# autonomousvision/unimatch

Measured on NVIDIA H100. Metric: image-pairs/sec @480x832 gmflow-scale2-refine6; EPE vs reference, higher is better.
Workload: dtype fp32

## Files before the change

### include/unimatch_sm100.h

```cpp
#ifndef UNIMATCH_SM100_H_
#define UNIMATCH_SM100_H_

#include <stdint.h>

#ifdef __cplusplus
extern "C" {
#endif

#define UM_OK 0
#define UM_EINVAL (-22)
#define UM_ECUDA (-5)

#define UM_FEATURE_DIM 128

#define UM_ABI_VERSION 4
int um_abi_version(void);
const char* um_build_info(void);
const char* um_last_error(void);
int64_t um_launch_count(void);

#define UM_MASK_NONE 0
#define UM_MASK_SWIN 1
#define UM_MASK_CAUSAL 2

typedef struct um_attn_geom {
  int32_t h, w;
  int32_t kh, kw;
  int32_t sh, sw;
  int32_t mask_mode;
} um_attn_geom;

int um_window_attention(const float* q, const float* k, const float* v, float* out,
                        int32_t n_streams, int32_t kv_shift,
                        int64_t ldq, int64_t ldk, int64_t ldv, int64_t ldo,
                        const um_attn_geom* geom, void* workspace, int64_t workspace_bytes, int32_t flags,
                        void* stream);
#define UM_ATTN_FORCE_CUDA_CORES 1
int64_t um_window_attention_workspace(const um_attn_geom* geom, int32_t n_streams);

int32_t um_attention_planes_lp(const um_attn_geom* geom);
int um_window_attention_planes(const void* q_planes, const void* k_planes, const void* v_planes, float* out, int64_t ldo,
                               void* out_split, int64_t split_plane_stride, int32_t n_streams, int32_t kv_shift,
                               const um_attn_geom* geom, void* stream);

#define UM_VALUE_TENSOR 0
#define UM_VALUE_COORDS 1
#define UM_VALUE_XCOORD 2
#define UM_POST_NONE 0
#define UM_POST_MINUS_OWN 1
#define UM_POST_OWN_MINUS 2

int um_softmax_expectation(const float* q, const float* k, const float* values, float* out,
                           int32_t n_streams, int32_t n_total, int32_t kv_shift,
                           int64_t ldq, int64_t ldk, int32_t vdim, int32_t value_mode, int32_t post_op,
                           const um_attn_geom* geom, void* workspace, int64_t workspace_bytes, int32_t flags,
                           void* stream);
int64_t um_softmax_expectation_workspace(const um_attn_geom* geom, int32_t n_total, int32_t value_mode);

int um_local_corr_softmax(const float* f0, const float* f1, float* flow,
                          int32_t batch, int32_t h, int32_t w, int32_t ry, int32_t rx, int32_t stereo,
                          void* stream);

int um_local_corr_volume(const float* f0, const float* f1, const float* flow, float* corr,
                         int32_t batch, int32_t h, int32_t w, int32_t radius, int32_t flow_dim, void* stream);

int um_flow_warp(const float* f, const float* flow, float* out,
// ... 211 lines not shown
```

### unimatch_b200/csrc/um_api.cu

```cuda
#include <stdarg.h>

#include <atomic>
#include <initializer_list>

#include <cuda_fp16.h>

#include "um_common.cuh"

namespace um {

static thread_local char g_err[512] = "";
static std::atomic<long long> g_launches{0};

void set_error(const char* fmt, ...) {
  va_list ap;
  va_start(ap, fmt);
  vsnprintf(g_err, sizeof(g_err), fmt, ap);
  va_end(ap);
}
void count_launch(int n) { g_launches.fetch_add(n, std::memory_order_relaxed); }

int window_attention_simt(const float* q, const float* k, const float* v, float* out, int n_streams, int kv_shift,
                          long long ldq, long long ldk, long long ldv, long long ldo, const Geom& g, cudaStream_t st);
bool attention_tc_supported(const Geom& g);
size_t attention_tc_workspace_bytes(const Geom& g, int n_streams);
int window_attention_tc(const float* q, const float* k, const float* v, float* out, int n_streams, int kv_shift,
                        long long ldq, long long ldk, long long ldv, long long ldo, const Geom& g, void* workspace,
                        cudaStream_t st);
int attention_planes_launch(const __half* wq, const __half* wk, const __half* wv, float* out, long long ldo, __half* out_split,
                            long long split_plane, int n_streams, int kv_shift, const Geom& g, cudaStream_t st);
bool expectation_tc_supported(const Geom& g, int value_mode);
size_t expectation_tc_workspace_bytes(const Geom& g, int n_total);
int softmax_expectation_tc(const float* q, const float* k, const float* values, float* out, int n_streams, int n_total,
                           int kv_shift, long long ldq, long long ldk, int vdim, int value_mode, int post_op,
                           const Geom& g, void* workspace, cudaStream_t st);
int softmax_expectation_simt(const float* q, const float* k, const float* values, float* out, int n_streams,
                             int n_total, int kv_shift, long long ldq, long long ldk, int vdim, int value_mode,
                             int post_op, const Geom& g, cudaStream_t st);
int chain_tracks_launch(const float* flow, const float* occ, int n, int h, int w, float* pos, uint8_t* vis, float* pos_out,
                        uint8_t* vis_out, cudaStream_t st);
int track_points_forward_launch(const float* flow, const float* occ, int n, int h, int w, int t0, const float* queries,
                                int nq, int nt, float* pos, uint8_t* vis, float* tracks, uint8_t* visible, cudaStream_t st);
int track_points_backward_launch(const float* flow, const float* occ, int n, int h, int w, const float* queries, int nq,
                                 int nt, float* tracks, uint8_t* visible, cudaStream_t st);

static bool overlap(const void* a, long long abytes, const void* b, long long bbytes) {
  const uintptr_t x = reinterpret_cast<uintptr_t>(a), y = reinterpret_cast<uintptr_t>(b);
  return x < y + (uintptr_t)bbytes && y < x + (uintptr_t)abytes;
}

struct Span {
  const void* p;
  long long bytes;
// ... 33 lines not shown
  um::Geom g;
  if (!um::make_geom(geom, &g) || !um::attention_tc_supported(g)) return 0;
  return (g.lw + 127) / 128 * 128;
}

int um_window_attention_planes(const void* q_planes, const void* k_planes, const void* v_planes, float* out, int64_t ldo,
                               void* out_split, int64_t split_plane_stride, int32_t n_streams, int32_t kv_shift,
                               const um_attn_geom* geom, void* stream) {
  um::Geom g;
  UM_REQUIRE(q_planes && k_planes && v_planes && (out || out_split) && n_streams > 0,
             "um_window_attention_planes: null operand planes / no output / empty batch");
  UM_REQUIRE(um::make_geom(geom, &g), "um_window_attention_planes: bad geometry (h,w must be divisible by kh,kw)");
  UM_REQUIRE(um::attention_tc_supported(g),
             "um_window_attention_planes: geometry not built for the tensor-core kernel (um_attention_planes_lp() == 0)");
  UM_REQUIRE(kv_shift >= 0 && kv_shift < n_streams, "um_window_attention_planes: kv_shift out of range");
  UM_REQUIRE(!out || (ldo % 4 == 0 && ldo >= UM_C), "um_window_attention_planes: ldo must be >= 128 and a multiple of 4");
  UM_REQUIRE(!out_split || (split_plane_stride >= (int64_t)n_streams * g.h * g.w * UM_C && split_plane_stride % 8 == 0),
             "um_window_attention_planes: split_plane_stride must cover n_streams*h*w rows of 128 halves");
  UM_REQUIRE(((reinterpret_cast<uintptr_t>(q_planes) | reinterpret_cast<uintptr_t>(k_planes) |
               reinterpret_cast<uintptr_t>(v_planes) | reinterpret_cast<uintptr_t>(out_split)) & 15) == 0,
             "um_window_attention_planes: planes must be 16-byte aligned");
  return um::attention_planes_launch(reinterpret_cast<const __half*>(q_planes), reinterpret_cast<const __half*>(k_planes),
                                     reinterpret_cast<const __half*>(v_planes), out, ldo, reinterpret_cast<__half*>(out_split),
                                     split_plane_stride, n_streams, kv_shift, g, (cudaStream_t)stream);
}

int um_window_attention(const float* q, const float* k, const float* v, float* out, int32_t n_streams,
                        int32_t kv_shift, int64_t ldq, int64_t ldk, int64_t ldv, int64_t ldo,
                        const um_attn_geom* geom, void* workspace, int64_t workspace_bytes, int32_t flags,
                        void* stream) {
  um::Geom g;
  UM_REQUIRE(q && k && v && out && n_streams > 0, "um_window_attention: null pointer or empty batch");
  UM_REQUIRE(um::make_geom(geom, &g), "um_window_attention: bad geometry (h,w must be divisible by kh,kw)");
  UM_REQUIRE(kv_shift >= 0 && kv_shift < n_streams, "um_window_attention: kv_shift out of range");
  UM_REQUIRE(ldq % 4 == 0 && ldk % 4 == 0 && ldv % 4 == 0 && ldo % 4 == 0 && ldq >= UM_C && ldk >= UM_C &&
                 ldv >= UM_C && ldo >= UM_C,
             "um_window_attention: row strides must be >= 128 and multiples of 4 floats");
  UM_REQUIRE(g.mask_mode >= UM_MASK_NONE && g.mask_mode <= UM_MASK_CAUSAL, "um_window_attention: bad mask_mode");
  cudaStream_t st = (cudaStream_t)stream;
  if (!(flags & UM_ATTN_FORCE_CUDA_CORES) && um::attention_tc_supported(g)) {
    UM_REQUIRE(workspace && workspace_bytes >= (int64_t)um::attention_tc_workspace_bytes(g, n_streams),
               "um_window_attention: workspace too small (%lld bytes needed, see um_window_attention_workspace)",
               (long long)um::attention_tc_workspace_bytes(g, n_streams));
    return um::window_attention_tc(q, k, v, out, n_streams, kv_shift, ldq, ldk, ldv, ldo, g, workspace, st);
  }
  return um::window_attention_simt(q, k, v, out, n_streams, kv_shift, ldq, ldk, ldv, ldo, g, st);
}
// ... 90 lines not shown
```

### unimatch_b200/csrc/um_attention_tc.cu

```cuda
#include <math_constants.h>

#include "um_common.cuh"
#include "um_tc.cuh"

namespace um {

using namespace tc;

namespace {

constexpr int BM = 128, BN = 64;
constexpr int NTHREADS = 288;
constexpr int PRODUCER = 8;
constexpr uint32_t Q_BYTES = 4 * 16384;
constexpr uint32_t KV_STAGE_BYTES = 4 * 8192;
constexpr uint32_t OFF_Q = 0;
constexpr uint32_t OFF_K = OFF_Q + Q_BYTES;
constexpr uint32_t OFF_V = OFF_K + 2 * KV_STAGE_BYTES;
constexpr uint32_t OFF_X = OFF_V + 2 * KV_STAGE_BYTES;
constexpr uint32_t OFF_BAR = OFF_X + 1024;
constexpr uint32_t OFF_KREG = OFF_BAR + 256;
constexpr int MAX_LP = 2048;
constexpr uint32_t SMEM_BYTES = OFF_KREG + MAX_LP;
constexpr float SQRT_C = 11.313708498984761f;
constexpr float EXP_SCALE = 1.4426950408889634f / 11.313708498984761f;
constexpr float LAZY_THRESH = 8.0f / EXP_SCALE;

struct TcParams {
  float* out; long long ldo;
  int n_streams, kv_shift, lp;
  Geom g;
  const float* values; int vdim, value_mode, post_op;
  __half* out_split; long long split_plane;
};

__device__ __forceinline__ uint32_t pack_h2(__half a, __half b) {
  return (uint32_t)__half_as_ushort(a) | ((uint32_t)__half_as_ushort(b) << 16);
}

template <bool HAS_V>
__global__ void __launch_bounds__(NTHREADS, 1)
attn_tc_kernel(const __grid_constant__ CUtensorMap map_q, const __grid_constant__ CUtensorMap map_k,
               const __grid_constant__ CUtensorMap map_v, TcParams p) {
  extern __shared__ __align__(1024) uint8_t smem[];
  uint64_t* bars = reinterpret_cast<uint64_t*>(smem + OFF_BAR);
  uint64_t* q_full = bars + 0;
  uint64_t* k_full = bars + 1;
  uint64_t* k_empty = bars + 3;
  uint64_t* v_full = bars + 5;
  uint64_t* v_empty = bars + 7;
  int8_t* kreg = reinterpret_cast<int8_t*>(smem + OFF_KREG);

  const Geom g = p.g;
  const int warp = threadIdx.x >> 5, lane = threadIdx.x & 31;
  const int m0 = blockIdx.x * BM, win = blockIdx.y, n = blockIdx.z;
  const int nk = (n + p.kv_shift) % p.n_streams;
  const int nwin = g.nwin, lp = p.lp;
  const int T = (g.lw + BN - 1) / BN;
  const int planes = p.n_streams * nwin * lp;

  if (threadIdx.x == 0) {
    mbar_init(q_full, 1);
    for (int i = 0; i < 2; ++i) {
      mbar_init(k_full + i, 1); mbar_init(k_empty + i, 8);
      mbar_init(v_full + i, 1); mbar_init(v_empty + i, 8);
    }
// ... 229 lines not shown
    fence_acc(o);
    __syncwarp();
    if (lane == 0) mbar_arrive(v_empty + s);
  }

  float inv[2];
#pragma unroll
  for (int h = 0; h < 2; ++h) {
    float l = l_run[h];
    l += __shfl_xor_sync(0xffffffffu, l, 1);
    l += __shfl_xor_sync(0xffffffffu, l, 2);
    inv[h] = 1.0f / l;
  }
  consumers_sync();
  float* osm = reinterpret_cast<float*>(smem + OFF_Q);
#pragma unroll
  for (int jj = 0; jj < 16; ++jj)
#pragma unroll
    for (int h = 0; h < 2; ++h) {
      const int row = fr + 8 * h, col = 8 * jj + fc;
      *reinterpret_cast<float2*>(osm + row * 128 + (((col >> 2) ^ (row & 31)) << 2) + (col & 3)) =
          make_float2(o[4 * jj + 2 * h] * inv[h], o[4 * jj + 2 * h + 1] * inv[h]);
    }
  consumers_sync();
  float* obase = p.out + (long long)n * g.h * g.w * p.ldo;
  for (int row = cw * 16; row < cw * 16 + 16; ++row) {
    const int tq = m0 + row;
    if (tq >= g.lw) break;
    const int tk = window_token(g, win, tq);
    const float4 v = *reinterpret_cast<const float4*>(osm + row * 128 + ((lane ^ (row & 31)) << 2));
    if (p.out) *reinterpret_cast<float4*>(obase + (long long)tk * p.ldo + lane * 4) = v;
    if (p.out_split) {
      uint32_t h0, h1, l0, l1;
      split_f16x2(v.x, v.y, &h0, &l0);
      split_f16x2(v.z, v.w, &h1, &l1);
      __half* d = p.out_split + ((long long)n * g.h * g.w + tk) * 128 + lane * 4;
      *reinterpret_cast<uint2*>(d) = make_uint2(h0, h1);
      *reinterpret_cast<uint2*>(d + p.split_plane) = make_uint2(l0, l1);
    }
  }
}

struct SplitParams {
  const float* src[3]; long long ld[3];
  __half* dst[3];
  int n_streams, lp;
  Geom g;
};

__global__ void __launch_bounds__(256) split_windows_kernel(SplitParams p) {
  const Geom g = p.g;
  const int lane = threadIdx.x & 31;
  const int t = blockIdx.x * 8 + (threadIdx.x >> 5);
  const int win = blockIdx.y, n = blockIdx.z;
  if (t >= p.lp) return;
  const long long planes = (long long)p.n_streams * g.nwin * p.lp;
  const long long row = ((long long)n * g.nwin + win) * p.lp + t;
  const int tok = (t < g.lw) ? window_token(g, win, t) : -1;
#pragma unroll
  for (int a = 0; a < 3; ++a) {
    if (!p.src[a]) continue;
// ... 49 lines not shown
}

bool attention_tc_supported(const Geom& g) {
  return g.lw >= BM && padded_lw(g.lw) <= MAX_LP && (g.mask_mode == UM_MASK_NONE || g.mask_mode == UM_MASK_SWIN);
}

size_t attention_tc_workspace_bytes(const Geom& g, int n_streams) {
  return (size_t)3 * 2 * n_streams * g.nwin * padded_lw(g.lw) * 128 * sizeof(__half);
}

int split_windows_launch(const float* q, const float* k, const float* v, long long ldq, long long ldk, long long ldv,
                         __half* wq, __half* wk, __half* wv, int n_streams, const Geom& g, cudaStream_t st, const char* what) {
  SplitParams sp{};
  sp.src[0] = q; sp.src[1] = k; sp.src[2] = v;
  sp.ld[0] = ldq; sp.ld[1] = ldk; sp.ld[2] = ldv;
  sp.dst[0] = wq; sp.dst[1] = wk; sp.dst[2] = wv;
  sp.n_streams = n_streams; sp.lp = padded_lw(g.lw); sp.g = g;
  split_windows_kernel<<<dim3((sp.lp + 7) / 8, g.nwin, n_streams), 256, 0, st>>>(sp);
  return check_launch(what);
}


int attention_planes_launch(const __half* wq, const __half* wk, const __half* wv, float* out, long long ldo, __half* out_split,
                               long long split_plane, int n_streams, int kv_shift, const Geom& g, cudaStream_t st) {
  const int lp = padded_lw(g.lw);
  int rc;
  CUtensorMap mq, mk, mv;
  const uint64_t rows = (uint64_t)2 * n_streams * g.nwin * lp;
  if ((rc = make_map_2d_f16(&mq, wq, rows, 128, BM))) return rc;
  if ((rc = make_map_2d_f16(&mk, wk, rows, 128, BN))) return rc;
  if ((rc = make_map_2d_f16(&mv, wv, rows, 128, BN))) return rc;
  static PerDeviceBytes configured;
  if ((rc = ensure_smem(configured, attn_tc_kernel<true>, SMEM_BYTES, "attn_tc"))) return rc;
  TcParams p{};
  p.out = out; p.ldo = ldo; p.n_streams = n_streams; p.kv_shift = kv_shift; p.lp = lp; p.g = g;
  p.out_split = out_split; p.split_plane = split_plane;
  const int qtiles = (g.lw + BM - 1) / BM;
  attn_tc_kernel<true><<<dim3(qtiles, g.nwin, n_streams), NTHREADS, SMEM_BYTES, st>>>(mq, mk, mv, p);
  return check_launch("um_window_attention(wgmma)");
}

int window_attention_tc(const float* q, const float* k, const float* v, float* out, int n_streams, int kv_shift,
                        long long ldq, long long ldk, long long ldv, long long ldo, const Geom& g, void* workspace,
                        cudaStream_t st) {
  const int lp = padded_lw(g.lw);
  const size_t plane_elems = (size_t)2 * n_streams * g.nwin * lp * 128;
  __half* wq = reinterpret_cast<__half*>(workspace);
  __half* wk = wq + plane_elems;
  __half* wv = wk + plane_elems;
  int rc = split_windows_launch(q, k, v, ldq, ldk, ldv, wq, wk, wv, n_streams, g, st, "um_window_attention(split)");
  if (rc) return rc;
  return attention_planes_launch(wq, wk, wv, out, ldo, nullptr, 0, n_streams, kv_shift, g, st);
}

int softmax_expectation_tc(const float* q, const float* k, const float* values, float* out, int n_streams, int n_total,
                           int kv_shift, long long ldq, long long ldk, int vdim, int value_mode, int post_op,
                           const Geom& g, void* workspace, cudaStream_t st) {
  const int lp = padded_lw(g.lw);
  const size_t plane_elems = (size_t)2 * n_total * g.nwin * lp * 128;
  __half* wq = reinterpret_cast<__half*>(workspace);
  __half* wk = wq + plane_elems;
  int rc = split_windows_launch(q, k, nullptr, ldq, ldk, 0, wq, wk, nullptr, n_total, g, st, "um_softmax_expectation(split)");
  if (rc) return rc;
  CUtensorMap mq, mk;
  const uint64_t rows = (uint64_t)2 * n_total * g.nwin * lp;
  if ((rc = make_map_2d_f16(&mq, wq, rows, 128, BM))) return rc;
  if ((rc = make_map_2d_f16(&mk, wk, rows, 128, BN))) return rc;
  static PerDeviceBytes configured;
  if ((rc = ensure_smem(configured, attn_tc_kernel<false>, SMEM_BYTES, "expect_tc"))) return rc;
  TcParams p{};
  p.out = out; p.ldo = vdim; p.n_streams = n_total; p.kv_shift = kv_shift; p.lp = lp; p.g = g;
  p.values = values; p.vdim = vdim; p.value_mode = value_mode; p.post_op = post_op;
  const int qtiles = (g.lw + BM - 1) / BM;
  attn_tc_kernel<false><<<dim3(qtiles, g.nwin, n_streams), NTHREADS, SMEM_BYTES, st>>>(mq, mk, mk, p);
  return check_launch("um_softmax_expectation(wgmma)");
// ... 4 lines not shown
```

### unimatch_b200/csrc/um_common.cuh

```cuda
#pragma once
#include <cuda_runtime.h>
#include <stdint.h>
#include <stdio.h>

#include "unimatch_sm100.h"

#define UM_STR2(x) #x
#define UM_STR(x) UM_STR2(x)
#define UM_C 128

namespace um {

void set_error(const char* fmt, ...);
void count_launch(int n = 1);

inline int check_launch(const char* what) {
  cudaError_t e = cudaGetLastError();
  if (e != cudaSuccess) {
    set_error("%s: %s", what, cudaGetErrorString(e));
    return UM_ECUDA;
  }
  count_launch();
  return UM_OK;
}
// ... 20 lines not shown
inline int device_sm_count() {
  static int sms[kMaxDevices] = {};
  const int d = current_device();
  if (!sms[d]) {
    int n = 0;
    cudaDeviceGetAttribute(&n, cudaDevAttrMultiProcessorCount, d);
    sms[d] = n > 0 ? n : 132;
  }
  return sms[d];
}

#define UM_REQUIRE(cond, ...)             \
  do {                                    \
    if (!(cond)) {                        \
      um::set_error(__VA_ARGS__);         \
      return UM_EINVAL;                   \
    }                                     \
  } while (0)

struct Geom {
  int h, w, kh, kw, wh, ww, sh, sw, mask_mode, lw, nwin;
};

inline bool make_geom(const um_attn_geom* g, Geom* o) {
  if (!g || g->h <= 0 || g->w <= 0 || g->kh <= 0 || g->kw <= 0) return false;
  if (g->h % g->kh || g->w % g->kw) return false;
  o->h = g->h; o->w = g->w; o->kh = g->kh; o->kw = g->kw;
  o->wh = g->h / g->kh; o->ww = g->w / g->kw;
  o->sh = g->sh; o->sw = g->sw; o->mask_mode = g->mask_mode;
  o->lw = o->wh * o->ww; o->nwin = g->kh * g->kw;
  if (o->sh < 0 || o->sh >= o->h || o->sw < 0 || o->sw >= o->w) return false;
  return true;
}

__device__ __forceinline__ int window_token(const Geom& g, int win, int t, int* yr_out = nullptr, int* xr_out = nullptr) {
  int wy = win / g.kw, wx = win - wy * g.kw;
  int i = t / g.ww, j = t - i * g.ww;
  int yr = wy * g.wh + i, xr = wx * g.ww + j;
  if (yr_out) *yr_out = yr;
  if (xr_out) *xr_out = xr;
  int y = yr + g.sh; if (y >= g.h) y -= g.h;
  int x = xr + g.sw; if (x >= g.w) x -= g.w;
  return y * g.w + x;
}

__device__ __forceinline__ int shift_region(const Geom& g, int yr, int xr) {
// ... 24 lines not shown
```

### unimatch_b200/ops.py

```python
import ctypes
import os

import torch

_HERE = os.path.dirname(os.path.abspath(__file__))
LIB_PATH = os.path.join(_HERE, "libunimatch_sm100.so")

MASK_NONE, MASK_SWIN, MASK_CAUSAL = 0, 1, 2
VALUE_TENSOR, VALUE_COORDS, VALUE_XCOORD = 0, 1, 2
POST_NONE, POST_MINUS_OWN, POST_OWN_MINUS = 0, 1, 2


FORCE_CUDA_CORES = 1
_force_cuda_cores = False


def set_force_cuda_cores(flag):
    global _force_cuda_cores
    _force_cuda_cores = bool(flag)


EVAL_FLOW, EVAL_STEREO, EVAL_DEPTH = 0, 1, 2
EVAL_MASK_ALL, EVAL_MASK_VALID, EVAL_MASK_VALID_MAX = 0, 1, 2
EVAL_PARTS = 128
# ... 39 lines not shown
RAGGED_ITEM_BYTES = ctypes.sizeof(RaggedItem)


class FfnDesc(ctypes.Structure):
    _fields_ = [("src", ctypes.c_void_p * 2), ("src_plane_stride", ctypes.c_int64), ("rows", ctypes.c_int64),
                ("w1", ctypes.c_void_p), ("w2", ctypes.c_void_p), ("hidden", ctypes.c_int32),
                ("residual", ctypes.c_void_p), ("ld_res", ctypes.c_int64), ("gamma", ctypes.c_void_p), ("beta", ctypes.c_void_p),
                ("out_f32", ctypes.c_void_p), ("ld_f32", ctypes.c_int64), ("out_split", ctypes.c_void_p),
                ("split_plane_stride", ctypes.c_int64)]


_P, _I, _L, _F = ctypes.c_void_p, ctypes.c_int32, ctypes.c_int64, ctypes.c_float
_G, _FP, _RC = ctypes.POINTER(AttnGeom), ctypes.POINTER(ctypes.c_float), ctypes.c_int

_SIGNATURES = {
    "um_abi_version": (_RC, []),
    "um_build_info": (ctypes.c_char_p, []),
    "um_last_error": (ctypes.c_char_p, []),
    "um_launch_count": (_L, []),
    "um_window_attention": (_RC, [_P, _P, _P, _P, _I, _I, _L, _L, _L, _L, _G, _P, _L, _I, _P]),
    "um_window_attention_workspace": (_L, [_G, _I]),
    "um_attention_planes_lp": (_I, [_G]),
    "um_window_attention_planes": (_RC, [_P, _P, _P, _P, _L, _P, _L, _I, _I, _G, _P]),
    "um_softmax_expectation": (_RC, [_P, _P, _P, _P, _I, _I, _I, _L, _L, _I, _I, _I, _G, _P, _L, _I, _P]),
    "um_softmax_expectation_workspace": (_L, [_G, _I, _I]),
    "um_local_corr_softmax": (_RC, [_P, _P, _P, _I, _I, _I, _I, _I, _I, _P]),
    "um_local_corr_volume": (_RC, [_P, _P, _P, _P, _I, _I, _I, _I, _I, _P]),
    "um_flow_warp": (_RC, [_P, _P, _P, _I, _I, _I, _I, _P]),
    "um_fb_consistency": (_RC, [_P, _P, _F, _F, _P, _P, _I, _I, _I, _P]),
    "um_fb_consistency_ragged": (_RC, [_P, _L, _P, _F, _F, _P, _L, _P, _I, _I, _I, _P]),
    "um_chain_tracks": (_RC, [_P, _P, _I, _I, _I, _P, _P, _P, _P, _P]),
    "um_track_points_forward": (_RC, [_P, _P, _I, _I, _I, _I, _P, _I, _I, _P, _P, _P, _P, _P]),
    "um_track_points_backward": (_RC, [_P, _P, _I, _I, _I, _P, _I, _I, _P, _P, _P]),
    "um_propagate_local": (_RC, [_P, _P, _P, _P, _I, _I, _I, _I, _I, _L, _L, _P]),
    "um_depth_corr_softmax": (_RC, [_P, _P, _P, _P, _P, _P, _P, _I, _I, _I, _I, _I, _P]),
    "um_add_position": (_RC, [_P, _P, _P, _I, _I, _I, _I, _I, _P]),
    "um_convex_upsample": (_RC, [_P, _P, _P, _I, _I, _I, _I, _I, _F, _P]),
    "um_upsample2x": (_RC, [_P, _P, _I, _I, _I, _I, _F, _P]),
    "um_resize_bilinear": (_RC, [_P, _P, _I, _I, _I, _I, _I, _I, _FP, _I, _P]),
    "um_frames_to_planar": (_RC, [_P, _P, _I, _I, _I, _I, _I, _I, _P]),
    "um_frames_to_planar_ragged": (_RC, [_P, _L, _P, _P, _I, _I, _I, _I, _I, _P]),
    "um_frames_to_planar_normalized": (_RC, [_P, _P, _I, _I, _I, _I, _I, _FP, _FP, _P]),
    "um_frames_to_planar_normalized_ragged": (_RC, [_P, _L, _P, _P, _I, _I, _I, _I, _I, _FP, _FP, _P]),
    "um_resize_bilinear_ragged": (_RC, [_P, _P, _L, _P, _I, _I, _I, _I, _I, _P]),
    "um_disparity_to_image_ragged": (_RC, [_P, _L, _P, _P, _P, _I, _I, _I, _P]),
    "um_flow_to_image": (_RC, [_P, _P, _L, _L, _P, _I, _I, _I, _P]),
# ... 117 lines not shown

def _window_attention_planes(qp, kp, vp, n, kv_shift, h, w, kh, kw, sh, sw, mask_mode, out_f32, out_split):
    g = AttnGeom(h, w, kh, kw, sh, sw, mask_mode)
    lp = int(LIB.um_attention_planes_lp(ctypes.byref(g)))
    if lp == 0:
        raise RuntimeError("window_attention_planes: geometry is not built for the tensor-core kernel")
    for t, nm in ((qp, "q_planes"), (kp, "k_planes"), (vp, "v_planes")):
        _planes_ok(t, nm, n, kh * kw, lp)
    ldo, plane = 0, 0
    if out_f32 is not None:
        ldo = _rows(out_f32, "out_f32")
    if out_split is not None:
        if out_split.dtype != torch.float16 or not out_split.is_contiguous() or out_split.shape[0] != 2 or out_split.shape[-1] != 128:
            raise RuntimeError("window_attention_planes: out_split must be contiguous fp16 planes [2, rows, 128]")
        plane = out_split[0].numel()
    _check(LIB.um_window_attention_planes(_p(qp), _p(kp), _p(vp), _p(out_f32), ldo, _p(out_split), plane, n, kv_shift,
                                          ctypes.byref(g), _stream()), "um_window_attention_planes")


window_attention_planes = _define(
    "window_attention_planes(Tensor q_planes, Tensor k_planes, Tensor v_planes, int n_streams, int kv_shift, int h, int w, "
    "int kh, int kw, int sh, int sw, int mask_mode, Tensor(a!)? out_f32, Tensor(b!)? out_split) -> ()",
    _window_attention_planes)


def _softmax_expectation(q, k, values, n_streams, kv_shift, vdim, value_mode, post_op, h, w, kh, kw, mask_mode):
    ldq, ldk = _rows(q, "q"), _rows(k, "k")
    n_total, l, _ = q.shape
    if values is not None:
        _f32c(values, "values")
    out = torch.empty((n_streams, l, vdim), device=q.device, dtype=torch.float32)
    g = AttnGeom(h, w, kh, kw, 0, 0, mask_mode)
    flags = FORCE_CUDA_CORES if _force_cuda_cores else 0
    ws_bytes = 0 if flags else int(LIB.um_softmax_expectation_workspace(ctypes.byref(g), n_total, value_mode))
    ws = torch.empty((ws_bytes,), device=q.device, dtype=torch.uint8) if ws_bytes else None
    _check(LIB.um_softmax_expectation(_p(q), _p(k), _p(values), _p(out), n_streams, n_total, kv_shift, ldq, ldk, vdim,
                                      value_mode, post_op, ctypes.byref(g), _p(ws), ws_bytes, flags, _stream()),
           "um_softmax_expectation")
    return out


softmax_expectation = _define(
    "softmax_expectation(Tensor q, Tensor k, Tensor? values, int n_streams, int kv_shift, int vdim, int value_mode, "
    "int post_op, int h, int w, int kh, int kw, int mask_mode) -> Tensor", _softmax_expectation)


# ... 646 lines not shown
```

### unimatch_b200/unimatch.py

```python
import math
from collections import namedtuple
from contextlib import contextmanager

import torch
import torch.nn as nn

from . import ops
from .spec import param_spec

_OPS = torch.ops.unimatch_sm100


class _Layer(namedtuple("_Layer", "weights bias kh kw pad_h pad_w stride cout bn mode act gamma beta k")):
    __slots__ = ()

    def out_hw(self, h, w, stride):
        return (h + 2 * self.pad_h - self.kh) // stride + 1, (w + 2 * self.pad_w - self.kw) // stride + 1


def _layer(w, cin_splits, bn, bias=None, act=ops.ACT_NONE, mode=ops.CONV_LINEAR, gamma=None, beta=None, stride=1):
    if w.dim() == 2:
        w = w[:, :, None, None]
    cout, cin, kh, kw = w.shape
    return _Layer(ops.prep_conv_weight(w, cin_splits, (cout + bn - 1) // bn * bn), bias, kh, kw, kh // 2, kw // 2, stride,
# ... 72 lines not shown
        elif ".norm" in key:
            t.fill_(1.0 if key.endswith("weight") else 0.0)
        else:
            t.uniform_(-0.05, 0.05)
        return t

    def train(self, mode=True):
        if mode:
            raise NotImplementedError("unimatch_b200.UniMatch is inference-only (use .eval(); training stays on the reference)")
        return super().train(False)

    def _prepared(self):
        params = dict(self.named_parameters())
        key = (tuple((p._version, p.data_ptr()) for p in params.values()),)
        if self._prep_key == key:
            return self._prep
        w = {k: v.detach() for k, v in params.items()}
        LN = ops.CONV_LN
        P = {"raw": w, "blocks": []}
        for i in range(self.num_transformer_layers):
            sk, ck = "transformer.layers.%d.self_attn." % i, "transformer.layers.%d.cross_attn_ffn." % i
            w_in = torch.cat([w[sk + "q_proj.weight"], w[sk + "k_proj.weight"], w[sk + "v_proj.weight"],
                              w[ck + "k_proj.weight"], w[ck + "v_proj.weight"]], dim=0)
            hid = w[ck + "mlp.0.weight"].shape[0]
            P["blocks"].append(dict(
                tc_in=_layer(w_in, [128], 128),
                tc_m_s=_layer(w[sk + "merge.weight"], [128], 128, mode=LN, gamma=w[sk + "norm1.weight"], beta=w[sk + "norm1.bias"]),
                tc_q_c=_layer(w[ck + "q_proj.weight"], [128], 128),
                tc_m_c=_layer(w[ck + "merge.weight"], [128], 128, mode=LN, gamma=w[ck + "norm1.weight"], beta=w[ck + "norm1.bias"]),
                tc_w1=_layer(w[ck + "mlp.0.weight"], [128, 128], 256, act=ops.ACT_GELU),
                tc_w2=_layer(w[ck + "mlp.2.weight"], [hid], 128, mode=LN, gamma=w[ck + "norm2.weight"], beta=w[ck + "norm2.bias"])))
        P["tcb"] = self._prepare_backbone(w, self.num_scales)
        qw, qb = w["feature_flow_attn.q_proj.weight"], w["feature_flow_attn.q_proj.bias"]
        kw, kb = w["feature_flow_attn.k_proj.weight"], w["feature_flow_attn.k_proj.bias"]
        P["prop_q"] = _layer(qw, [128], 128, qb.contiguous())
        P["prop_k"] = _layer(kw, [128], 128, kb.contiguous())
        P["prop_qk"] = _layer(torch.cat([qw, kw], 0), [128], 128, torch.cat([qb, kb]).contiguous())
        if self.reg_refine:
            P["tc"] = self._prepare_refine(w)
        if "upsampler.0.weight" in w:
            w0 = w["upsampler.0.weight"]
            w0 = torch.cat([w0[:, 2:], w0[:, :2]], dim=1)
            w2 = w["upsampler.2.weight"]
            P["up"] = dict(c0=_layer(w0, [130], 128, w["upsampler.0.bias"], act=ops.ACT_RELU),
                           c2=_layer(w2, [256], 192 if w2.shape[0] % 192 == 0 else 64, w["upsampler.2.bias"]))
        self._prep_key, self._prep = key, P
        return P

    @staticmethod
# ... 181 lines not shown
        if buf is None:
            if len(self._attn_ws) >= 4:
                self._attn_ws.clear()
            buf = torch.zeros((6, 2, n, kh * kw, lp, 128), device=dev, dtype=torch.float16)
            self._attn_ws[key] = buf
        return buf

    def cached_buffers(self):
        return list(self._attn_ws.values()) + list(self._pad_ws.values())

    def _stage_transformer(self, P, x, h, w, attn_type, splits, tag="s0"):
        n, l, c = x.shape
        half = n // 2
        rows = n * l
        rp = _ceil16(rows)
        dev = x.device
        G = self._conv
        mk = torch.empty if rp == rows else torch.zeros
        planes = lambda cp: mk((2, rp, cp), device=dev, dtype=torch.float16)
        f32 = lambda cols: mk((rp, cols), device=dev)
        tok = lambda t, c0, c1: t[:rows].view(n, l, t.shape[-1])[:, :, c0:c1]
        hid = P["blocks"][0]["tc_w1"].cout
        x_f, xo_f, x1_f = f32(c), f32(c), f32(c)
        x_s, xo_s, x1_s, msg_s, m_s = planes(c), planes(c), planes(c), planes(c), planes(c)
        fused_ffn = ops.ffn_tc_supported(rp)
        hid_s = None if fused_ffn else planes(hid)
        x_f[:rows] = x.reshape(rows, c)
        _OPS.split_planes(x_f, x_s, 0)
        y = q_f = None
        for i, blk in enumerate(P["blocks"]):
            geo_s, geo_c = self._attn_plan(attn_type, splits, h, w, i)
            gs, gc = (h, w) + geo_s, (h, w) + geo_c
            lp_s = ops.attention_planes_lp(*gs)
            lp_c = ops.attention_planes_lp(*gc) if geo_c == geo_s else 0
            ws = self._attn_planes(dev, n, h, w, geo_s[0], geo_s[1], lp_s) if lp_s else None
            win_c1 = 640 if lp_c else (384 if lp_s else 0)
            if win_c1 < 640 and y is None:
                y = f32(5 * c)
            G(blk["tc_in"], x_s, rows=rp, out_f32=y if win_c1 < 640 else None, win_dst=ws[:win_c1 // 128] if win_c1 else None,
              win_geom=gs if win_c1 else None, win_c1=win_c1, win_streams=n)
            fl_s, fl_c = (4.0 * (l // (g[0] * g[1])) * l * 128 * n for g in (geo_s, geo_c))
            if lp_s:
                self._timed("attn:" + tag, fl_s, _OPS.window_attention_planes, ws[0], ws[1], ws[2], n, 0, *gs, None, msg_s)
            else:
                msg = self._timed("attn_simt:" + tag, fl_s, _OPS.window_attention, tok(y, 0, 128), tok(y, 128, 256), tok(y, 256, 384), 0, *gs)
                _OPS.split_planes(msg.view(rows, c), msg_s, 0)
            G(blk["tc_m_s"], msg_s, rows=rp, out_f32=x1_f, out_split=x1_s, aux0=x_f)
            if lp_c:
                G(blk["tc_q_c"], x1_s, rows=rp, win_dst=ws[5:6], win_geom=gc, win_c1=128, win_streams=n)
                self._timed("attn:" + tag, fl_c, _OPS.window_attention_planes, ws[5], ws[3], ws[4], n, half, *gc, None, msg_s)
            else:
                if q_f is None:
                    q_f = f32(c)
                G(blk["tc_q_c"], x1_s, rows=rp, out_f32=q_f)
                msg = self._timed("attn_simt:" + tag, fl_c, _OPS.window_attention, tok(q_f, 0, 128), tok(y, 384, 512), tok(y, 512, 640), half, *gc)
                _OPS.split_planes(msg.view(rows, c), msg_s, 0)
            G(blk["tc_m_c"], msg_s, rows=rp, out_split=m_s)
            w1, w2 = blk["tc_w1"], blk["tc_w2"]
            if fused_ffn:
                self._timed("conv", 2.0 * rp * hid * (2 * c + c), _OPS.ffn_tc, x1_s, m_s, w1.weights, w2.weights, x1_f,
                            w2.gamma, w2.beta, xo_f, xo_s, rp)
            else:
                G(w1, x1_s, m_s, rows=rp, out_split=hid_s)
                G(w2, hid_s, rows=rp, out_f32=xo_f, out_split=xo_s, aux0=x1_f)
            x_f, xo_f, x_s, xo_s = xo_f, x_f, xo_s, x_s
        return x_f[:rows].view(n, l, c), x_s

    def _stage_features(self, f0, f1, flow, h, wd, splits):
        Bp, c = f0.shape[0], f0.shape[-1]
        if flow is not None:
            f1 = _OPS.flow_warp(f1.contiguous(), flow.contiguous(), h, wd)
        table = self._pos_table(h // splits, wd // splits, f0.device)
        tok = torch.cat((f0, f1), dim=0).view(2 * Bp, h, wd, c)
        return _OPS.add_position(tok, table, h, wd).view(2 * Bp, h * wd, c)

    def _stage_correlation(self, tok, Bp, h, wd, task, radius, pred_bidir_flow=False, depth=None):
        t0, t1 = tok[:Bp], tok[Bp:]
        if task == "depth":
            cams, from_argmax, bidir = depth
            if bidir:
# ... 280 lines not shown
```

Before: 82.51.

## Fold merge and cross-query projections into weights and fuse LayerNorm into attention

Two weight products are precomputed in fp64 and stored with the fused input projection: merge·v_proj for self and cross attention, and q_proj^T·k_proj for cross attention. The separate merge and cross-query GEMMs disappear from each transformer block. A new attention kernel variant applies LayerNorm, the residual add and split-fp16 output, including a windowed layout that feeds the next attention, directly in its epilogue. This removes several GEMM launches and intermediate buffers per block, at the cost of a heavier epilogue and some numerical drift from the pre-multiplied weights.

```diff
diff --git a/include/unimatch_sm100.h b/include/unimatch_sm100.h
--- a/include/unimatch_sm100.h
+++ b/include/unimatch_sm100.h
@@ -42,6 +42,10 @@
 int um_window_attention_planes(const void* q_planes, const void* k_planes, const void* v_planes, float* out, int64_t ldo,
                                void* out_split, int64_t split_plane_stride, int32_t n_streams, int32_t kv_shift,
                                const um_attn_geom* geom, void* stream);
+int um_window_attention_planes_ln(const void* q_planes, const void* k_planes, const void* v_planes, const float* residual,
+                                  int64_t ld_res, const float* gamma, const float* beta, float* out, int64_t ldo,
+                                  void* out_split, int64_t split_plane_stride, void* out_win, int32_t n_streams,
+                                  int32_t kv_shift, const um_attn_geom* geom, void* stream);
 
 #define UM_VALUE_TENSOR 0
 #define UM_VALUE_COORDS 1
diff --git a/unimatch_b200/csrc/um_api.cu b/unimatch_b200/csrc/um_api.cu
--- a/unimatch_b200/csrc/um_api.cu
+++ b/unimatch_b200/csrc/um_api.cu
@@ -28,7 +28,8 @@
                         long long ldq, long long ldk, long long ldv, long long ldo, const Geom& g, void* workspace,
                         cudaStream_t st);
 int attention_planes_launch(const __half* wq, const __half* wk, const __half* wv, float* out, long long ldo, __half* out_split,
-                            long long split_plane, int n_streams, int kv_shift, const Geom& g, cudaStream_t st);
+                            long long split_plane, int n_streams, int kv_shift, const Geom& g, cudaStream_t st,
+                            const AttnEpilogue& ep);
 bool expectation_tc_supported(const Geom& g, int value_mode);
 size_t expectation_tc_workspace_bytes(const Geom& g, int n_total);
 int softmax_expectation_tc(const float* q, const float* k, const float* values, float* out, int n_streams, int n_total,
@@ -108,7 +109,41 @@
              "um_window_attention_planes: planes must be 16-byte aligned");
   return um::attention_planes_launch(reinterpret_cast<const __half*>(q_planes), reinterpret_cast<const __half*>(k_planes),
                                      reinterpret_cast<const __half*>(v_planes), out, ldo, reinterpret_cast<__half*>(out_split),
-                                     split_plane_stride, n_streams, kv_shift, g, (cudaStream_t)stream);
+                                     split_plane_stride, n_streams, kv_shift, g, (cudaStream_t)stream, um::AttnEpilogue{});
+}
+
+int um_window_attention_planes_ln(const void* q_planes, const void* k_planes, const void* v_planes, const float* residual,
+                                  int64_t ld_res, const float* gamma, const float* beta, float* out, int64_t ldo,
+                                  void* out_split, int64_t split_plane_stride, void* out_win, int32_t n_streams,
+                                  int32_t kv_shift, const um_attn_geom* geom, void* stream) {
+  um::Geom g;
+  UM_REQUIRE(q_planes && k_planes && v_planes && gamma && beta && (out || out_split || out_win) && n_streams > 0,
+             "um_window_attention_planes_ln: null operand planes / gamma / beta, no output or empty batch");
+  UM_REQUIRE(um::make_geom(geom, &g), "um_window_attention_planes_ln: bad geometry (h,w must be divisible by kh,kw)");
+  UM_REQUIRE(um::attention_tc_supported(g),
+             "um_window_attention_planes_ln: geometry not built for the tensor-core kernel (um_attention_planes_lp() == 0)");
+  UM_REQUIRE(kv_shift >= 0 && kv_shift < n_streams, "um_window_attention_planes_ln: kv_shift out of range");
+  UM_REQUIRE(!out || (ldo % 4 == 0 && ldo >= UM_C), "um_window_attention_planes_ln: ldo must be >= 128 and a multiple of 4");
+  UM_REQUIRE(!residual || (ld_res % 4 == 0 && ld_res >= UM_C),
+             "um_window_attention_planes_ln: ld_res must be >= 128 and a multiple of 4");
+  UM_REQUIRE(!out_split || (split_plane_stride >= (int64_t)n_streams * g.h * g.w * UM_C && split_plane_stride % 8 == 0),
+             "um_window_attention_planes_ln: split_plane_stride must cover n_streams*h*w rows of 128 halves");
+  UM_REQUIRE(um::aligned(q_planes, 16) && um::aligned(k_planes, 16) && um::aligned(v_planes, 16) && um::aligned(out_split, 16) &&
+             um::aligned(out_win, 16) && um::aligned(out, 16) && um::aligned(residual, 16) && um::aligned(gamma, 16) &&
+             um::aligned(beta, 16), "um_window_attention_planes_ln: buffers must be 16-byte aligned");
+  const long long rows = (long long)n_streams * g.h * g.w;
+  const long long win_halves = 2LL * n_streams * g.nwin * ((g.lw + 127) / 128 * 128) * UM_C;
+  UM_REQUIRE(um::written_disjoint({{out, out ? ((rows - 1) * ldo + UM_C) * 4 : 0},
+                                   {out_split, out_split ? (split_plane_stride + rows * UM_C) * 2 : 0},
+                                   {out_win, win_halves * 2},
+                                   {residual, residual ? ((rows - 1) * ld_res + UM_C) * 4 : 0},
+                                   {q_planes, win_halves * 2}, {k_planes, win_halves * 2}, {v_planes, win_halves * 2}}, 3),
+             "um_window_attention_planes_ln: an output overlaps another output or an input");
+  um::AttnEpilogue ep;
+  ep.gamma = gamma; ep.beta = beta; ep.residual = residual; ep.ldr = ld_res; ep.out_win = reinterpret_cast<__half*>(out_win);
+  return um::attention_planes_launch(reinterpret_cast<const __half*>(q_planes), reinterpret_cast<const __half*>(k_planes),
+                                     reinterpret_cast<const __half*>(v_planes), out, ldo, reinterpret_cast<__half*>(out_split),
+                                     split_plane_stride, n_streams, kv_shift, g, (cudaStream_t)stream, ep);
 }
 
 int um_window_attention(const float* q, const float* k, const float* v, float* out, int32_t n_streams,
diff --git a/unimatch_b200/csrc/um_attention_tc.cu b/unimatch_b200/csrc/um_attention_tc.cu
--- a/unimatch_b200/csrc/um_attention_tc.cu
+++ b/unimatch_b200/csrc/um_attention_tc.cu
@@ -1,4 +1,6 @@
 #include <math_constants.h>
+
+#include <type_traits>
 
 #include "um_common.cuh"
 #include "um_tc.cuh"
@@ -34,14 +36,21 @@
   __half* out_split; long long split_plane;
 };
 
+struct TcFoldParams : TcParams {
+  const float* gamma; const float* beta;
+  const float* residual; long long ldr;
+  __half* out_win;
+};
+
 __device__ __forceinline__ uint32_t pack_h2(__half a, __half b) {
   return (uint32_t)__half_as_ushort(a) | ((uint32_t)__half_as_ushort(b) << 16);
 }
 
-template <bool HAS_V>
+template <bool HAS_V, typename Params = TcParams>
 __global__ void __launch_bounds__(NTHREADS, 1)
 attn_tc_kernel(const __grid_constant__ CUtensorMap map_q, const __grid_constant__ CUtensorMap map_k,
-               const __grid_constant__ CUtensorMap map_v, TcParams p) {
+               const __grid_constant__ CUtensorMap map_v, Params p) {
+  constexpr bool FOLDED = std::is_same<Params, TcFoldParams>::value;
   extern __shared__ __align__(1024) uint8_t smem[];
   uint64_t* bars = reinterpret_cast<uint64_t*>(smem + OFF_BAR);
   uint64_t* q_full = bars + 0;
@@ -317,21 +326,70 @@
       *reinterpret_cast<float2*>(osm + row * 128 + (((col >> 2) ^ (row & 31)) << 2) + (col & 3)) =
           make_float2(o[4 * jj + 2 * h] * inv[h], o[4 * jj + 2 * h + 1] * inv[h]);
     }
+  const int row0 = cw * 16;
+  float4 res[FOLDED ? 16 : 1];
+  if constexpr (FOLDED) {
+    if (p.residual) {
+#pragma unroll
+      for (int i = 0; i < 16; ++i) {
+        const int tq = m0 + row0 + i;
+        res[i] = tq < g.lw ? __ldg(reinterpret_cast<const float4*>(p.residual + ((long long)n * g.h * g.w +
+                                                                                 window_token(g, win, tq)) * p.ldr) + lane)
+                           : make_float4(0.f, 0.f, 0.f, 0.f);
+      }
+    }
+  }
   consumers_sync();
   float* obase = p.out + (long long)n * g.h * g.w * p.ldo;
-  for (int row = cw * 16; row < cw * 16 + 16; ++row) {
-    const int tq = m0 + row;
-    if (tq >= g.lw) break;
-    const int tk = window_token(g, win, tq);
-    const float4 v = *reinterpret_cast<const float4*>(osm + row * 128 + ((lane ^ (row & 31)) << 2));
-    if (p.out) *reinterpret_cast<float4*>(obase + (long long)tk * p.ldo + lane * 4) = v;
-    if (p.out_split) {
-      uint32_t h0, h1, l0, l1;
-      split_f16x2(v.x, v.y, &h0, &l0);
-      split_f16x2(v.z, v.w, &h1, &l1);
-      __half* d = p.out_split + ((long long)n * g.h * g.w + tk) * 128 + lane * 4;
-      *reinterpret_cast<uint2*>(d) = make_uint2(h0, h1);
-      *reinterpret_cast<uint2*>(d + p.split_plane) = make_uint2(l0, l1);
+  if constexpr (!FOLDED) {
+    for (int row = cw * 16; row < cw * 16 + 16; ++row) {
+      const int tq = m0 + row;
+      if (tq >= g.lw) break;
+      const int tk = window_token(g, win, tq);
+      const float4 v = *reinterpret_cast<const float4*>(osm + row * 128 + ((lane ^ (row & 31)) << 2));
+      if (p.out) *reinterpret_cast<float4*>(obase + (long long)tk * p.ldo + lane * 4) = v;
+      if (p.out_split) {
+        uint32_t h0, h1, l0, l1;
+        split_f16x2(v.x, v.y, &h0, &l0);
+        split_f16x2(v.z, v.w, &h1, &l1);
+        __half* d = p.out_split + ((long long)n * g.h * g.w + tk) * 128 + lane * 4;
+        *reinterpret_cast<uint2*>(d) = make_uint2(h0, h1);
+        *reinterpret_cast<uint2*>(d + p.split_plane) = make_uint2(l0, l1);
+      }
+    }
+  } else {
+    const float4 gam = __ldg(reinterpret_cast<const float4*>(p.gamma) + lane);
+    const float4 bet = __ldg(reinterpret_cast<const float4*>(p.beta) + lane);
+#pragma unroll
+    for (int i = 0; i < 16; ++i) {
+      const int row = row0 + i, tq = m0 + row;
+      if (tq >= g.lw) break;
+      const int tk = window_token(g, win, tq);
+      float4 v = *reinterpret_cast<const float4*>(osm + row * 128 + ((lane ^ (row & 31)) << 2));
+      const float mean = warp_sum((v.x + v.y) + (v.z + v.w)) * (1.0f / 128.0f);
+      v.x -= mean; v.y -= mean; v.z -= mean; v.w -= mean;
+      const float var = warp_sum(fmaf(v.x, v.x, fmaf(v.y, v.y, fmaf(v.z, v.z, v.w * v.w)))) * (1.0f / 128.0f);
+      const float rstd = rsqrtf(var + 1e-5f);
+      v.x = fmaf(v.x * rstd, gam.x, bet.x); v.y = fmaf(v.y * rstd, gam.y, bet.y);
+      v.z = fmaf(v.z * rstd, gam.z, bet.z); v.w = fmaf(v.w * rstd, gam.w, bet.w);
+      if (p.residual) { v.x += res[i].x; v.y += res[i].y; v.z += res[i].z; v.w += res[i].w; }
+      if (p.out) *reinterpret_cast<float4*>(obase + (long long)tk * p.ldo + lane * 4) = v;
+      if (p.out_win) {
+        uint32_t h0, h1, l0, l1;
+        split_f16x2(v.x, v.y, &h0, &l0);
+        split_f16x2(v.z, v.w, &h1, &l1);
+        __half* d = p.out_win + ((long long)(n * nwin + win) * lp + tq) * 128 + lane * 4;
+        *reinterpret_cast<uint2*>(d) = make_uint2(h0, h1);
+        *reinterpret_cast<uint2*>(d + (long long)planes * 128) = make_uint2(l0, l1);
+      }
+      if (p.out_split) {
+        uint32_t h0, h1, l0, l1;
+        split_f16x2(v.x, v.y, &h0, &l0);
+        split_f16x2(v.z, v.w, &h1, &l1);
+        __half* d = p.out_split + ((long long)n * g.h * g.w + tk) * 128 + lane * 4;
+        *reinterpret_cast<uint2*>(d) = make_uint2(h0, h1);
+        *reinterpret_cast<uint2*>(d + p.split_plane) = make_uint2(l0, l1);
+      }
     }
   }
 }
@@ -427,7 +485,8 @@
 
 
 int attention_planes_launch(const __half* wq, const __half* wk, const __half* wv, float* out, long long ldo, __half* out_split,
-                               long long split_plane, int n_streams, int kv_shift, const Geom& g, cudaStream_t st) {
+                               long long split_plane, int n_streams, int kv_shift, const Geom& g, cudaStream_t st,
+                               const AttnEpilogue& ep) {
   const int lp = padded_lw(g.lw);
   int rc;
   CUtensorMap mq, mk, mv;
@@ -435,13 +494,20 @@
   if ((rc = make_map_2d_f16(&mq, wq, rows, 128, BM))) return rc;
   if ((rc = make_map_2d_f16(&mk, wk, rows, 128, BN))) return rc;
   if ((rc = make_map_2d_f16(&mv, wv, rows, 128, BN))) return rc;
-  static PerDeviceBytes configured;
-  if ((rc = ensure_smem(configured, attn_tc_kernel<true>, SMEM_BYTES, "attn_tc"))) return rc;
-  TcParams p{};
+  static PerDeviceBytes configured, configured_folded;
+  TcFoldParams p{};
   p.out = out; p.ldo = ldo; p.n_streams = n_streams; p.kv_shift = kv_shift; p.lp = lp; p.g = g;
   p.out_split = out_split; p.split_plane = split_plane;
   const int qtiles = (g.lw + BM - 1) / BM;
-  attn_tc_kernel<true><<<dim3(qtiles, g.nwin, n_streams), NTHREADS, SMEM_BYTES, st>>>(mq, mk, mv, p);
+  const dim3 grid(qtiles, g.nwin, n_streams);
+  if (ep.gamma) {
+    if ((rc = ensure_smem(configured_folded, attn_tc_kernel<true, TcFoldParams>, SMEM_BYTES, "attn_tc(folded)"))) return rc;
+    p.gamma = ep.gamma; p.beta = ep.beta; p.residual = ep.residual; p.ldr = ep.ldr; p.out_win = ep.out_win;
+    attn_tc_kernel<true, TcFoldParams><<<grid, NTHREADS, SMEM_BYTES, st>>>(mq, mk, mv, p);
+  } else {
+    if ((rc = ensure_smem(configured, attn_tc_kernel<true>, SMEM_BYTES, "attn_tc"))) return rc;
+    attn_tc_kernel<true><<<grid, NTHREADS, SMEM_BYTES, st>>>(mq, mk, mv, static_cast<const TcParams&>(p));
+  }
   return check_launch("um_window_attention(wgmma)");
 }
 
@@ -455,7 +521,7 @@
   __half* wv = wk + plane_elems;
   int rc = split_windows_launch(q, k, v, ldq, ldk, ldv, wq, wk, wv, n_streams, g, st, "um_window_attention(split)");
   if (rc) return rc;
-  return attention_planes_launch(wq, wk, wv, out, ldo, nullptr, 0, n_streams, kv_shift, g, st);
+  return attention_planes_launch(wq, wk, wv, out, ldo, nullptr, 0, n_streams, kv_shift, g, st, AttnEpilogue{});
 }
 
 int softmax_expectation_tc(const float* q, const float* k, const float* values, float* out, int n_streams, int n_total,
diff --git a/unimatch_b200/csrc/um_common.cuh b/unimatch_b200/csrc/um_common.cuh
--- a/unimatch_b200/csrc/um_common.cuh
+++ b/unimatch_b200/csrc/um_common.cuh
@@ -1,4 +1,5 @@
 #pragma once
+#include <cuda_fp16.h>
 #include <cuda_runtime.h>
 #include <stdint.h>
 #include <stdio.h>
@@ -66,6 +67,12 @@
   int h, w, kh, kw, wh, ww, sh, sw, mask_mode, lw, nwin;
 };
 
+struct AttnEpilogue {
+  const float* gamma = nullptr; const float* beta = nullptr;
+  const float* residual = nullptr; long long ldr = 0;
+  __half* out_win = nullptr;
+};
+
 inline bool make_geom(const um_attn_geom* g, Geom* o) {
   if (!g || g->h <= 0 || g->w <= 0 || g->kh <= 0 || g->kw <= 0) return false;
   if (g->h % g->kh || g->w % g->kw) return false;
diff --git a/unimatch_b200/ops.py b/unimatch_b200/ops.py
--- a/unimatch_b200/ops.py
+++ b/unimatch_b200/ops.py
@@ -85,6 +85,7 @@
     "um_window_attention_workspace": (_L, [_G, _I]),
     "um_attention_planes_lp": (_I, [_G]),
     "um_window_attention_planes": (_RC, [_P, _P, _P, _P, _L, _P, _L, _I, _I, _G, _P]),
+    "um_window_attention_planes_ln": (_RC, [_P, _P, _P, _P, _L, _P, _P, _P, _L, _P, _L, _P, _I, _I, _G, _P]),
     "um_softmax_expectation": (_RC, [_P, _P, _P, _P, _I, _I, _I, _L, _L, _I, _I, _I, _G, _P, _L, _I, _P]),
     "um_softmax_expectation_workspace": (_L, [_G, _I, _I]),
     "um_local_corr_softmax": (_RC, [_P, _P, _P, _I, _I, _I, _I, _I, _I, _P]),
@@ -248,6 +249,52 @@
     "window_attention_planes(Tensor q_planes, Tensor k_planes, Tensor v_planes, int n_streams, int kv_shift, int h, int w, "
     "int kh, int kw, int sh, int sw, int mask_mode, Tensor(a!)? out_f32, Tensor(b!)? out_split) -> ()",
     _window_attention_planes)
+
+
+def has_kernel(op_name, device):
+    key = "CUDA" if torch.device(device).type == "cuda" else "CPU"
+    return torch._C._dispatch_has_kernel_for_dispatch_key("unimatch_sm100::" + op_name, key)
+
+
+def _token_rows(t, name, rows):
+    _f32c(t, name, rows_ok=True)
+    if t.shape[-1] != 128 or t.numel() < rows * 128:
+        raise RuntimeError("%s: expected >= %d fp32 rows of 128 channels" % (name, rows))
+    ld = t.stride(-2) if t.dim() >= 2 else 128
+    if t.dim() >= 3 and t.stride(-3) != ld * t.shape[-2]:
+        raise RuntimeError("%s: rows must be equally spaced" % name)
+    return ld
+
+
+def _window_attention_planes_ln(qp, kp, vp, n, kv_shift, h, w, kh, kw, sh, sw, mask_mode, residual, gamma, beta, out_f32,
+                                out_split, out_win):
+    g = AttnGeom(h, w, kh, kw, sh, sw, mask_mode)
+    lp = int(LIB.um_attention_planes_lp(ctypes.byref(g)))
+    if lp == 0:
+        raise RuntimeError("window_attention_planes_ln: geometry is not built for the tensor-core kernel")
+    for t, nm in ((qp, "q_planes"), (kp, "k_planes"), (vp, "v_planes")) + (((out_win, "out_win"),) if out_win is not None else ()):
+        _planes_ok(t, nm, n, kh * kw, lp)
+    for t, nm in ((gamma, "gamma"), (beta, "beta")):
+        _f32c(t, nm)
+        if t.numel() != 128:
+            raise RuntimeError("window_attention_planes_ln: %s must hold 128 floats" % nm)
+    rows = n * h * w
+    ldr = _token_rows(residual, "residual", rows) if residual is not None else 0
+    ldo = _token_rows(out_f32, "out_f32", rows) if out_f32 is not None else 0
+    plane = 0
+    if out_split is not None:
+        if out_split.dtype != torch.float16 or not out_split.is_contiguous() or out_split.shape[0] != 2 or out_split.shape[-1] != 128:
+            raise RuntimeError("window_attention_planes_ln: out_split must be contiguous fp16 planes [2, rows, 128]")
+        plane = out_split[0].numel()
+    _check(LIB.um_window_attention_planes_ln(_p(qp), _p(kp), _p(vp), _p(residual), ldr, _p(gamma), _p(beta), _p(out_f32), ldo,
+                                             _p(out_split), plane, _p(out_win), n, kv_shift, ctypes.byref(g), _stream()),
+           "um_window_attention_planes_ln")
+
+
+window_attention_planes_ln = _define(
+    "window_attention_planes_ln(Tensor q_planes, Tensor k_planes, Tensor v_planes, int n_streams, int kv_shift, int h, int w, "
+    "int kh, int kw, int sh, int sw, int mask_mode, Tensor? residual, Tensor gamma, Tensor beta, Tensor(a!)? out_f32, "
+    "Tensor(b!)? out_split, Tensor(c!)? out_win) -> ()", _window_attention_planes_ln)
 
 
 def _softmax_expectation(q, k, values, n_streams, kv_shift, vdim, value_mode, post_op, h, w, kh, kw, mask_mode):
diff --git a/unimatch_b200/unimatch.py b/unimatch_b200/unimatch.py
--- a/unimatch_b200/unimatch.py
+++ b/unimatch_b200/unimatch.py
@@ -118,9 +118,15 @@
             sk, ck = "transformer.layers.%d.self_attn." % i, "transformer.layers.%d.cross_attn_ffn." % i
             w_in = torch.cat([w[sk + "q_proj.weight"], w[sk + "k_proj.weight"], w[sk + "v_proj.weight"],
                               w[ck + "k_proj.weight"], w[ck + "v_proj.weight"]], dim=0)
+            f64 = lambda k: w[k].double()
+            w_fold = torch.cat([w[sk + "q_proj.weight"], w[sk + "k_proj.weight"],
+                                (f64(sk + "merge.weight") @ f64(sk + "v_proj.weight")).float(),
+                                (f64(ck + "q_proj.weight").t() @ f64(ck + "k_proj.weight")).float(),
+                                (f64(ck + "merge.weight") @ f64(ck + "v_proj.weight")).float()], dim=0)
             hid = w[ck + "mlp.0.weight"].shape[0]
             P["blocks"].append(dict(
                 tc_in=_layer(w_in, [128], 128),
+                tc_in_fold=_layer(w_fold, [128], 128),
                 tc_m_s=_layer(w[sk + "merge.weight"], [128], 128, mode=LN, gamma=w[sk + "norm1.weight"], beta=w[sk + "norm1.bias"]),
                 tc_q_c=_layer(w[ck + "q_proj.weight"], [128], 128),
                 tc_m_c=_layer(w[ck + "merge.weight"], [128], 128, mode=LN, gamma=w[ck + "norm1.weight"], beta=w[ck + "norm1.bias"]),
@@ -348,40 +354,51 @@
         tok = lambda t, c0, c1: t[:rows].view(n, l, t.shape[-1])[:, :, c0:c1]
         hid = P["blocks"][0]["tc_w1"].cout
         x_f, xo_f, x1_f = f32(c), f32(c), f32(c)
-        x_s, xo_s, x1_s, msg_s, m_s = planes(c), planes(c), planes(c), planes(c), planes(c)
+        x_s, xo_s, x1_s, m_s = planes(c), planes(c), planes(c), planes(c)
         fused_ffn = ops.ffn_tc_supported(rp)
         hid_s = None if fused_ffn else planes(hid)
         x_f[:rows] = x.reshape(rows, c)
         _OPS.split_planes(x_f, x_s, 0)
-        y = q_f = None
+        y = q_f = msg_s = None
+        can_fold = ops.has_kernel("window_attention_planes_ln", dev)
         for i, blk in enumerate(P["blocks"]):
             geo_s, geo_c = self._attn_plan(attn_type, splits, h, w, i)
             gs, gc = (h, w) + geo_s, (h, w) + geo_c
             lp_s = ops.attention_planes_lp(*gs)
             lp_c = ops.attention_planes_lp(*gc) if geo_c == geo_s else 0
             ws = self._attn_planes(dev, n, h, w, geo_s[0], geo_s[1], lp_s) if lp_s else None
-            win_c1 = 640 if lp_c else (384 if lp_s else 0)
-            if win_c1 < 640 and y is None:
-                y = f32(5 * c)
-            G(blk["tc_in"], x_s, rows=rp, out_f32=y if win_c1 < 640 else None, win_dst=ws[:win_c1 // 128] if win_c1 else None,
-              win_geom=gs if win_c1 else None, win_c1=win_c1, win_streams=n)
             fl_s, fl_c = (4.0 * (l // (g[0] * g[1])) * l * 128 * n for g in (geo_s, geo_c))
-            if lp_s:
-                self._timed("attn:" + tag, fl_s, _OPS.window_attention_planes, ws[0], ws[1], ws[2], n, 0, *gs, None, msg_s)
+            ms, mc = blk["tc_m_s"], blk["tc_m_c"]
+            if lp_c and can_fold:
+                G(blk["tc_in_fold"], x_s, rows=rp, win_dst=ws[:5], win_geom=gs, win_c1=640, win_streams=n)
+                self._timed("attn:" + tag, fl_s, _OPS.window_attention_planes_ln, ws[0], ws[1], ws[2], n, 0, *gs, x_f,
+                            ms.gamma, ms.beta, x1_f, x1_s, ws[5])
+                self._timed("attn:" + tag, fl_c, _OPS.window_attention_planes_ln, ws[5], ws[3], ws[4], n, half, *gc, None,
+                            mc.gamma, mc.beta, None, m_s, None)
             else:
-                msg = self._timed("attn_simt:" + tag, fl_s, _OPS.window_attention, tok(y, 0, 128), tok(y, 128, 256), tok(y, 256, 384), 0, *gs)
-                _OPS.split_planes(msg.view(rows, c), msg_s, 0)
-            G(blk["tc_m_s"], msg_s, rows=rp, out_f32=x1_f, out_split=x1_s, aux0=x_f)
-            if lp_c:
-                G(blk["tc_q_c"], x1_s, rows=rp, win_dst=ws[5:6], win_geom=gc, win_c1=128, win_streams=n)
-                self._timed("attn:" + tag, fl_c, _OPS.window_attention_planes, ws[5], ws[3], ws[4], n, half, *gc, None, msg_s)
-            else:
-                if q_f is None:
-                    q_f = f32(c)
-                G(blk["tc_q_c"], x1_s, rows=rp, out_f32=q_f)
-                msg = self._timed("attn_simt:" + tag, fl_c, _OPS.window_attention, tok(q_f, 0, 128), tok(y, 384, 512), tok(y, 512, 640), half, *gc)
-                _OPS.split_planes(msg.view(rows, c), msg_s, 0)
-            G(blk["tc_m_c"], msg_s, rows=rp, out_split=m_s)
+                win_c1 = 640 if lp_c else (384 if lp_s else 0)
+                if msg_s is None:
+                    msg_s = planes(c)
+                if win_c1 < 640 and y is None:
+                    y = f32(5 * c)
+                G(blk["tc_in"], x_s, rows=rp, out_f32=y if win_c1 < 640 else None, win_dst=ws[:win_c1 // 128] if win_c1 else None,
+                  win_geom=gs if win_c1 else None, win_c1=win_c1, win_streams=n)
+                if lp_s:
+                    self._timed("attn:" + tag, fl_s, _OPS.window_attention_planes, ws[0], ws[1], ws[2], n, 0, *gs, None, msg_s)
+                else:
+                    msg = self._timed("attn_simt:" + tag, fl_s, _OPS.window_attention, tok(y, 0, 128), tok(y, 128, 256), tok(y, 256, 384), 0, *gs)
+                    _OPS.split_planes(msg.view(rows, c), msg_s, 0)
+                G(ms, msg_s, rows=rp, out_f32=x1_f, out_split=x1_s, aux0=x_f)
+                if lp_c:
+                    G(blk["tc_q_c"], x1_s, rows=rp, win_dst=ws[5:6], win_geom=gc, win_c1=128, win_streams=n)
+                    self._timed("attn:" + tag, fl_c, _OPS.window_attention_planes, ws[5], ws[3], ws[4], n, half, *gc, None, msg_s)
+                else:
+                    if q_f is None:
+                        q_f = f32(c)
+                    G(blk["tc_q_c"], x1_s, rows=rp, out_f32=q_f)
+                    msg = self._timed("attn_simt:" + tag, fl_c, _OPS.window_attention, tok(q_f, 0, 128), tok(y, 384, 512), tok(y, 512, 640), half, *gc)
+                    _OPS.split_planes(msg.view(rows, c), msg_s, 0)
+                G(mc, msg_s, rows=rp, out_split=m_s)
             w1, w2 = blk["tc_w1"], blk["tc_w2"]
             if fused_ffn:
                 self._timed("conv", 2.0 * rp * hid * (2 * c + c), _OPS.ffn_tc, x1_s, m_s, w1.weights, w2.weights, x1_f,
```

Result: faster. 84.50, median of 6 (+2.4%).
